# arnaucube/go-snark-study

Measured on AMD Instinct MI355X. Metric: Groth16 constraints/sec (prove) at 2^20 R1CS, higher is better.
Workload: dtype u32 (9x29-bit Montgomery limbs of the 254-bit BN128 fields)

## Files before the change

go-snark-study_amd/csrc/knobs.h:

```cpp
#pragma once
#include <cerrno>
#include <cstdlib>

namespace gs {

inline bool knob_parse(const char* name, long lo, long hi, long multiple_of, bool pow2, long& out) {
  const char* s = getenv(name);
  if (!s || !*s) return false;
  char* end = nullptr;
  errno = 0;
  const long v = strtol(s, &end, 10);
  if (errno != 0 || end == s || *end != '\0') return false;
  if (v < lo || v > hi) return false;
  if (multiple_of > 1 && v % multiple_of != 0) return false;
  if (pow2 && (v <= 0 || (v & (v - 1)) != 0)) return false;
  out = v;
  return true;
}

inline bool run_flag(const char* name) { return getenv(name) != nullptr; }
inline long run_knob(const char* name, long dflt, long lo, long hi) {
  long v = dflt;
  return knob_parse(name, lo, hi, 1, false, v) ? v : dflt;
}

#ifdef GS_DEV_KNOBS
inline bool dev_flag(const char* name) { return getenv(name) != nullptr; }
inline long dev_knob(const char* name, long dflt, long lo, long hi, long multiple_of = 1, bool pow2 = false) {
  long v = dflt;
  return knob_parse(name, lo, hi, multiple_of, pow2, v) ? v : dflt;
}
inline double dev_knob_f(const char* name, double dflt, double lo, double hi) {
  const char* s = getenv(name);
  if (!s || !*s) return dflt;
  char* end = nullptr;
  const double v = strtod(s, &end);
  return (end == s || *end != '\0' || !(v >= lo && v <= hi)) ? dflt : v;
}
#else
inline bool dev_flag(const char*) { return false; }
inline long dev_knob(const char*, long dflt, long, long, long = 1, bool = false) { return dflt; }
inline double dev_knob_f(const char*, double dflt, double, double) { return dflt; }
#endif

}
```

go-snark-study_amd/csrc/msm.hip:

```cpp
#include "msm.h"
#include "hostcopy.h"

#include <algorithm>
#include <cmath>
#include <cstdlib>
#include <future>
#include <type_traits>

#include "msm_kernels.h"

namespace gs {

static_assert(sizeof(G1Xyzz) == PointIO<FqTag>::kXyzzWords * 4, "G1 XYZZ must be raw limbs");
static_assert(sizeof(G2Xyzz) == PointIO<Fq2Tag>::kXyzzWords * 4, "G2 XYZZ must be raw limbs");

static inline dim3 grid1(size_t n, int block = 256) { return dim3((unsigned)((n + block - 1) / block)); }

int choose_window_bits(uint32_t n, int forced) {
  if (forced >= 8 && forced <= kMaxWindowBits) return forced;
  static const double per_bucket = dev_knob_f("GS_WINDOW_COST_BUCKET", 6.0, 0.0, 64.0);
  static const int auto_max = (int)dev_knob("GS_AUTO_MAX_C", 17, 8, kMaxWindowBits);
  int best = 8;
  double best_cost = 1e300;
  for (int c = 8; c <= std::min(kMaxWindowBits, std::max(8, auto_max)); ++c) {
    const int W = 254 / c + 1;
    const double cost = (double)n * W + per_bucket * (double)(1u << (c - 1));
    if (cost < best_cost) { best_cost = cost; best = c; }
  }
  return best;
}

int choose_window_bits_free(uint32_t n, int forced) {
  if (forced) return std::min(kMaxFreeWindowBits, std::max(kMinFreeWindowBits, forced));
  static const double per_bucket = dev_knob_f("GS_WINDOW_COST_BUCKET_FREE", 3.0, 0.0, 64.0);
  int best = kMinFreeWindowBits;
  double best_cost = 1e300;
  for (int c = kMinFreeWindowBits; c <= kMaxFreeWindowBits; ++c) {
    const int W = 254 / c + 1;
    const double cost = (double)W * ((double)n + per_bucket * (double)(1u << (c - 1)));
    if (cost < best_cost) { best_cost = cost; best = c; }
  }
  return best;
}

static void exclusive_scan(Ctx& c, PlanBuffers& pb, const uint32_t* in, uint32_t* out, uint32_t n) {
  const uint32_t ntiles = (n + kScanTile - 1) / kScanTile;
  pb.tiles.ensure((size_t)ntiles * 4);
  pb.total.ensure(4);
  hipLaunchKernelGGL(k_scan_tiles, dim3(ntiles), dim3(kScanBlock), 0, c.stream, in, out, pb.tiles.as<uint32_t>(), n);
  hipLaunchKernelGGL(k_scan_tile_sums, dim3(1), dim3(1024), 0, c.stream, pb.tiles.as<uint32_t>(), ntiles, pb.total.as<uint32_t>());
  hipLaunchKernelGGL(k_scan_add, dim3(ntiles), dim3(kScanBlock), 0, c.stream, out, pb.tiles.as<uint32_t>(), n);
}

struct MsmState {
  PlanBuffers plan_slots[3 * Ctx::kSlots];
  DevBuf table_scratch;
  DevBuf table_scratch_bg;
  DevBuf upload_scratch;
  DevBuf upload_flag;
  bool lds_attr_set = false;
};
static MsmState& msm_state(Ctx& c) { return c.state<MsmState>(c.msm_state); }

static uint32_t choose_chunk(uint64_t entries, uint32_t nbuckets, const std::vector<LaunchShape>& users) {
  static const int forced = (int)dev_knob("GS_CHUNK", 0, 4, 1024, 4);
  if (forced >= 4 && forced % 4 == 0) return (uint32_t)forced;
  static const int forced_h = (int)dev_knob("GS_CHUNK_H", 0, 4, 1024, 4);
  if (forced_h && users.size() == 1 && users[0].njobs == 1 && !users[0].g2) return (uint32_t)forced_h;
  uint32_t chunk = entries >= (1ull << 27) ? 64u : entries >= (1ull << 23) ? 32u : 16u;
  while (chunk < 1024u && entries / std::max<uint32_t>(nbuckets, 1u) > 32ull * chunk) chunk *= 2;
  return chunk;
}

static uint32_t part_min_ranges() {
  static const uint32_t v = (uint32_t)dev_knob("GS_PART_MIN_R", 4, 2, 64);
  return v;
}
bool plan_partitions_first(int cbits) {
// ... 28 lines not shown
  plan.B = 1u << (plan.c - 1);
  plan.nbuckets = table_free ? (uint32_t)plan.W * plan.B : plan.B;
  plan.chunk = choose_chunk((uint64_t)n * plan.W, plan.nbuckets, users);
  plan.maxchunks = (uint32_t)(((size_t)n * plan.W + plan.chunk - 1) / plan.chunk) + 1;
  const size_t ncount = (size_t)plan.nbuckets + 1;
  PlanParams pp{};
  pp.n = n; pp.c = plan.c; pp.W = plan.W; pp.B = plan.B;
  pp.R = std::max<uint32_t>(1u, plan.B >> kRangeLog);
  pp.tf = table_free ? 1u : 0u;
  {
    const uint32_t want = std::max<uint32_t>(1u, 256u / (plan.W * pp.R));
    const uint32_t by_size = std::max<uint32_t>(1u, (n + 16383u) / 16384u);
    const uint32_t by_mem = std::max<uint32_t>(1u, (uint32_t)((64ull << 20) / ((uint64_t)plan.B * plan.W * 4)));
    pp.S = std::max<uint32_t>(1u, std::min(std::min<uint32_t>(16u, std::max<uint32_t>(want, 1u)), std::min(by_size, by_mem)));
    if (pp.R == 1 && !table_free) pp.S = std::max<uint32_t>(1u, std::min<uint32_t>(16u, by_size));
  }
  pp.slice = (n + pp.S - 1) / pp.S;
  pp.stride = (n + 63u) & ~63u;
  const bool wide = plan_partitions_first(plan.c);
  if (wide && term_index) throw HipError{hipErrorInvalidValue, "plans over a term list cannot be sorted partition-first (plan_partitions_first)", __LINE__};
  const uint32_t nparts = (uint32_t)plan.W * pp.R;
  if (wide && nparts > kMaxParts) throw HipError{hipErrorInvalidValue, "too many (window, range) partitions", __LINE__};
  if (!wide) pb.digits.ensure((size_t)std::max<uint32_t>(pp.stride, 64u) * plan.W * sizeof(digit_t));
  else {
    pb.recs.ensure(std::max<size_t>((size_t)n * plan.W, 1) * 8);
    pb.parts.ensure((size_t)(3 * kMaxParts + 4) * 4);
  }
  pb.hist.ensure((size_t)plan.B * plan.W * pp.S * 4);
  pb.totals.ensure(ncount * 4);
  pb.offsets.ensure(ncount * 4);
  pb.entries.ensure(((size_t)plan.maxchunks + 1) * plan.chunk * 4);
  pb.chunk_bucket.ensure((size_t)plan.maxchunks * 4);
  pb.heavy_list.ensure((size_t)plan.nbuckets * 4);
  pb.counters.ensure(16);
  const size_t lds = (size_t)std::min<uint32_t>(plan.B, kRangeBuckets) * 4;
  static const int sort_block = (int)dev_knob("GS_SORT_BLOCK", kSortBlock, 64, kSortBlock, 64);
  if (!ms.lds_attr_set) {
    GS_HIP(hipFuncSetAttribute(reinterpret_cast<const void*>(k_hist), hipFuncAttributeMaxDynamicSharedMemorySize, 128 * 1024));
    GS_HIP(hipFuncSetAttribute(reinterpret_cast<const void*>(k_scatter), hipFuncAttributeMaxDynamicSharedMemorySize, 128 * 1024));
    GS_HIP(hipFuncSetAttribute(reinterpret_cast<const void*>(k_hist_part), hipFuncAttributeMaxDynamicSharedMemorySize, 128 * 1024));
    GS_HIP(hipFuncSetAttribute(reinterpret_cast<const void*>(k_scatter_part), hipFuncAttributeMaxDynamicSharedMemorySize, 128 * 1024));
    ms.lds_attr_set = true;
  }
  GS_HIP(hipMemsetAsync(pb.totals.as<uint32_t>() + plan.nbuckets, 0, 4, c.stream));
  GS_HIP(hipMemsetAsync(pb.counters.p, 0, 16, c.stream));
  uint32_t* part_count = pb.parts.as<uint32_t>();
  uint32_t* part_base = part_count ? part_count + kMaxParts : nullptr;
  uint32_t* part_cursor = part_count ? part_base + kMaxParts + 4 : nullptr;
  if (n > 0 && wide) {
    GS_HIP(hipMemsetAsync(part_count, 0, (size_t)nparts * 4, c.stream));
    hipLaunchKernelGGL(k_part_count, grid1(n, kPartBlock), dim3(kPartBlock), 0, c.stream, scalars_dev, pp, part_count);
    hipLaunchKernelGGL(k_part_scan, dim3(1), dim3(64), 0, c.stream, part_count, nparts, part_base, part_cursor);
    hipLaunchKernelGGL(k_part_scatter, grid1(n, kPartBlock * kPartPerThread), dim3(kPartBlock), 0, c.stream, scalars_dev, pp, part_base, part_cursor,
                       pb.recs.as<uint2>());
    hipLaunchKernelGGL(k_hist_part, dim3(8 * pp.S * ((nparts + 7) / 8)), dim3(sort_block), lds, c.stream, pb.recs.as<uint2>(), part_base, pp, pb.hist.as<uint32_t>());
    hipLaunchKernelGGL(k_colscan, grid1(plan.B), dim3(256), 0, c.stream, pb.hist.as<uint32_t>(), pp, pb.totals.as<uint32_t>());
  } else if (n > 0) {
    hipLaunchKernelGGL(k_digits, grid1(n), dim3(256), 0, c.stream, scalars_dev, pp, pb.digits.as<digit_t>(), term_index, index_bias);
    hipLaunchKernelGGL(k_hist, dim3(plan.W, pp.S, pp.R), dim3(sort_block), lds, c.stream, pb.digits.as<digit_t>(), pp, pb.hist.as<uint32_t>());
    if (table_free) hipLaunchKernelGGL(k_colscan_windows, grid1(plan.nbuckets), dim3(256), 0, c.stream, pb.hist.as<uint32_t>(), pp, pb.totals.as<uint32_t>());
    else hipLaunchKernelGGL(k_colscan, grid1(plan.B), dim3(256), 0, c.stream, pb.hist.as<uint32_t>(), pp, pb.totals.as<uint32_t>());
  } else {
    GS_HIP(hipMemsetAsync(pb.totals.p, 0, ncount * 4, c.stream));
  }
  exclusive_scan(c, pb, pb.totals.as<uint32_t>(), pb.offsets.as<uint32_t>(), (uint32_t)ncount);
  if (n > 0) {
    if (wide) hipLaunchKernelGGL(k_scatter_part, dim3(8 * pp.S * ((nparts + 7) / 8)), dim3(sort_block), lds, c.stream, pb.recs.as<uint2>(), part_base, pp,
                                 pb.hist.as<uint32_t>(), pb.offsets.as<uint32_t>(), pb.entries.as<uint32_t>());
    else hipLaunchKernelGGL(k_scatter, dim3(plan.W, pp.S, pp.R), dim3(sort_block), lds, c.stream, pb.digits.as<digit_t>(), pp, pb.hist.as<uint32_t>(),
                            pb.offsets.as<uint32_t>(), pb.entries.as<uint32_t>(), term_index, index_bias);
    hipLaunchKernelGGL(k_chunk_map, grid1(plan.nbuckets), dim3(256), 0, c.stream, pb.offsets.as<uint32_t>(), plan.nbuckets, plan.chunk,
                       pb.chunk_bucket.as<uint32_t>(), pb.heavy_list.as<uint32_t>(), pb.counters.as<uint32_t>());
  }
  GS_HIP(hipGetLastError());
  plan.offsets = pb.offsets.as<uint32_t>();
  plan.entries = pb.entries.as<uint32_t>();
  plan.chunk_bucket = pb.chunk_bucket.as<uint32_t>();
  plan.heavy_list = pb.heavy_list.as<uint32_t>();
  plan.heavy_count = pb.counters.as<uint32_t>();
}

template <class T>
static void enqueue_table_slabs(hipStream_t stream, DevBuf& scratch, const uint32_t* src, size_t n, int cbits, DevBuf& rows, size_t first, size_t last,
                                size_t slab) {
  const int W = 254 / cbits + 1;
  if (first >= last) return;
  static const bool per_row = dev_flag("GS_TABLE_PER_ROW");
  if (per_row || W <= 2) {
    if (first == 0) hipLaunchKernelGGL(k_build_table<T>, grid1(n), dim3(256), 0, stream, src, (uint32_t)n, cbits, W, rows.as<uint32_t>());
  } else {
    constexpr size_t sw = PointIO<T>::kXyzzWords + PointIO<T>::kXyzzWords / 4;
    slab = std::min<size_t>(std::max<size_t>(slab, 1), n);
    scratch.ensure(slab * (size_t)(W - 1) * sw * 4);
    for (size_t at = first; at < last; at += slab) {
// ... 205 lines not shown
  if (out_bytes > Ctx::kPinnedBytes) throw HipError{hipErrorInvalidValue, "MSM result staging too small", __LINE__};
  p.stats_off = out_bytes - stats_bytes;
  AccJobs jobs{};
  DevBuf& outb = c.ws_out[ws_base % Ctx::kWsSets];
  outb.ensure(pair_bytes + final_bytes + stats_bytes);
  uint32_t* finals = outb.as<uint32_t>() + pair_bytes / 4;
  uint32_t* stats = finals + final_bytes / 4;
  for (int j = 0; j < njobs; ++j) {
    const BaseTable* t = bases[j].table;
    const uint32_t* points = nullptr;
    uint32_t row_stride = 0;
    if (plan.table_free) {
      if (!bases[j].points || bases[j].off + plan.n > bases[j].npoints)
        throw HipError{hipErrorInvalidValue, "MSM base array does not cover the plan", __LINE__};
      points = bases[j].points + bases[j].off * aw;
    } else {
      if (!t || t->c != plan.c || !t->rows.p || bases[j].off + plan.n > t->n)
        throw HipError{hipErrorInvalidValue, "MSM base table does not match the plan", __LINE__};
      points = t->rows.as<uint32_t>() + bases[j].off * aw;
      row_stride = (uint32_t)t->n;
    }
    DevBuf& bk = c.ws_buckets[(ws_base + j) % Ctx::kWsSets];
    DevBuf& mg = c.ws_chunks[(ws_base + j) % Ctx::kWsSets];
    DevBuf& pt = c.ws_partials[(ws_base + j) % Ctx::kWsSets];
    bk.ensure((size_t)plan.nbuckets * pw * 4);
    mg.ensure((size_t)plan.nbuckets * pw * 4);
    pt.ensure((size_t)plan.maxchunks * 2 * pw * 4);
    jobs.j[j] = AccJob{points, row_stride, bk.as<uint32_t>(), pt.as<uint32_t>(),
                       pt.as<uint32_t>() + (size_t)plan.maxchunks * pw, mg.as<uint32_t>(),
                       outb.as<uint32_t>() + (size_t)j * nblk * 2 * pw, finals + (size_t)j * pw};
  }
  p.tacc = std::make_shared<PhaseTimer>(c.stream);
  p.tker = std::make_shared<PhaseTimer>(c.stream);
  hipLaunchKernelGGL(k_bucket_accumulate<T>, dim3((plan.maxchunks + kAccBlock - 1) / kAccBlock, njobs), dim3(kAccBlock), 0, c.stream,
                     jobs, plan.offsets, plan.entries, plan.chunk_bucket, plan.nbuckets, plan.chunk);
  p.tker->stop();
  p.tacc->stop();
  hipStream_t ts = tail_stream ? tail_stream : c.stream;
  if (ts != c.stream) {
    hipEvent_t ev;
    GS_HIP(hipEventCreateWithFlags(&ev, hipEventDisableTiming));
    GS_HIP(hipEventRecord(ev, c.stream));
    GS_HIP(hipStreamWaitEvent(ts, ev, 0));
    GS_HIP(hipEventDestroy(ev));
  }
  p.tred = std::make_shared<PhaseTimer>(ts);
  static const long alone_below_log2 = dev_knob("GS_TAIL_ALONE_LOG2", 19, 0, 32);
  const bool alone = plan.n < (1ull << alone_below_log2);
  auto launch_tails = [&](auto alone_tag) {
    constexpr bool kAlone = decltype(alone_tag)::value;
    hipLaunchKernelGGL((k_heavy_combine<T, kAlone>), dim3(64, njobs), dim3(kHeavyBlock), 0, ts,
                       jobs, plan.offsets, plan.heavy_list, plan.heavy_count, plan.chunk);
    hipLaunchKernelGGL((k_heavy_finish<T, kAlone>), dim3(16, njobs), dim3(kHeavyBlock), 0, ts,
                       jobs, plan.offsets, plan.heavy_list, plan.heavy_count, plan.chunk);
    hipLaunchKernelGGL((k_bucket_combine<T, kAlone>), dim3((plan.nbuckets + 255) / 256, njobs), dim3(256), 0, ts, jobs, plan.offsets, plan.nbuckets,
                       plan.chunk, plan.heavy_count, stats);
    hipLaunchKernelGGL((k_block_reduce<T, kAlone>), dim3(nblk, njobs), dim3(kReduceBlock), 0, ts, jobs, plan.nbuckets, L);
    if (p.folded) {
      int log2_span = 0;
      while ((1u << log2_span) < (uint32_t)kReduceBlock * (uint32_t)L) ++log2_span;
      hipLaunchKernelGGL((k_pair_reduce<T, kAlone>), dim3(1, njobs), dim3(kReduceBlock), 0, ts, jobs, nblk, log2_span);
    }
  };
  if (alone) launch_tails(std::true_type{}); else launch_tails(std::false_type{});
  GS_HIP(hipGetLastError());
  GS_HIP(hipMemcpyAsync(c.pinned[slot], p.folded ? (const void*)finals : outb.p, out_bytes, hipMemcpyDeviceToHost, ts));
  p.pinned_slot = c.pinned[slot];
// ... 213 lines not shown
```

go-snark-study_amd/csrc/msm_kernels.h:

```cpp
#pragma once
#include <hip/hip_runtime.h>
#include <stdint.h>

#include "ec.h"
#include "point_io.h"

namespace gs {

struct PlanParams {
  uint32_t n;
  int c;
  int W;
  uint32_t B;
  uint32_t S;
  uint32_t slice;
  uint32_t stride;
  uint32_t R;
  uint32_t tf;
};
constexpr uint32_t kRangeLog = 15;
constexpr uint32_t kRangeBuckets = 1u << kRangeLog;

GS_HD int32_t next_digit(const uint32_t (&k)[8], const PlanParams& pp, int w, uint32_t& carry) {
  uint32_t raw = scalar_bits(k, w * pp.c, pp.c) + carry;
// ... 28 lines not shown
  if (i < n) {
    uint32_t acc = 0;
    if (a) for (uint32_t k = 0; k < wa; ++k) acc |= a[(size_t)i * wa + k];
    if (b) for (uint32_t k = 0; k < wb; ++k) acc |= b[(size_t)i * wb + k];
    finite = acc != 0;
  }
  if (finite) { atomicOr(&mask[i >> 5], 1u << (i & 31u)); atomicAdd(count, 1u); }
}

constexpr int kSortBlock = 1024;

__global__ void __launch_bounds__(kSortBlock) k_hist(const digit_t* __restrict__ digits, PlanParams pp, uint32_t* __restrict__ hist) {
  wave_priority<GS_PRIO_PLAN>();
  extern __shared__ uint32_t sh[];
  const uint32_t w = blockIdx.x, s = blockIdx.y, r = blockIdx.z;
  const uint32_t nb = min(pp.B, kRangeBuckets), base = r << kRangeLog;
  for (uint32_t b = threadIdx.x; b < nb; b += blockDim.x) sh[b] = 0;
  __syncthreads();
  const uint32_t lo = s * pp.slice, hi = min(pp.n, lo + pp.slice);
  const digit_t* row = digits + (size_t)w * pp.stride;
  const int32_t zero = (int32_t)pp.B - 1;
  for (uint32_t i = lo + threadIdx.x; i < hi; i += blockDim.x) {
    const int32_t d = (int32_t)row[i] - zero;
    if (d != 0) {
      const uint32_t b = (uint32_t)(d < 0 ? -d : d) - 1u;
      if ((b >> kRangeLog) == r) atomicAdd(&sh[b - base], 1u);
    }
  }
  __syncthreads();
  uint32_t* out = hist + ((size_t)w * pp.S + s) * pp.B + base;
  for (uint32_t b = threadIdx.x; b < nb; b += blockDim.x) out[b] = sh[b];
}

__global__ void __launch_bounds__(256) k_colscan(uint32_t* __restrict__ hist, PlanParams pp, uint32_t* __restrict__ totals) {
  wave_priority<GS_PRIO_PLAN>();
  const uint32_t b = blockIdx.x * blockDim.x + threadIdx.x;
  if (b >= pp.B) return;
  uint32_t* col = hist + b;
  const uint32_t nq = (uint32_t)pp.W * pp.S;
  uint32_t run = 0;
  for (uint32_t q = 0; q < nq; ++q) { const uint32_t t = col[(size_t)q * pp.B]; col[(size_t)q * pp.B] = run; run += t; }
  totals[b] = run;
}

__global__ void __launch_bounds__(256) k_colscan_windows(uint32_t* __restrict__ hist, PlanParams pp, uint32_t* __restrict__ totals) {
  wave_priority<GS_PRIO_PLAN>();
  const uint32_t i = blockIdx.x * blockDim.x + threadIdx.x;
  if (i >= (uint32_t)pp.W * pp.B) return;
  const uint32_t w = i / pp.B, b = i % pp.B;
  uint32_t* col = hist + (size_t)w * pp.S * pp.B + b;
  uint32_t run = 0;
  for (uint32_t q = 0; q < pp.S; ++q) { const uint32_t t = col[(size_t)q * pp.B]; col[(size_t)q * pp.B] = run; run += t; }
  totals[i] = run;
}

__global__ void __launch_bounds__(kSortBlock) k_scatter(const digit_t* __restrict__ digits, PlanParams pp, const uint32_t* __restrict__ hist,
                                                         const uint32_t* __restrict__ offsets, uint32_t* __restrict__ entries,
                                                         const uint32_t* __restrict__ term_index, uint32_t index_bias) {
  wave_priority<GS_PRIO_PLAN>();
  extern __shared__ uint32_t sh[];
  const uint32_t w = blockIdx.x, s = blockIdx.y, r = blockIdx.z;
  const uint32_t nb = min(pp.B, kRangeBuckets), base = r << kRangeLog;
  const uint32_t* pre = hist + ((size_t)w * pp.S + s) * pp.B + base;
  const uint32_t* off = offsets + (pp.tf ? (size_t)w * pp.B : (size_t)0);
  for (uint32_t b = threadIdx.x; b < nb; b += blockDim.x) sh[b] = off[base + b] + pre[b];
  __syncthreads();
  const uint32_t lo = s * pp.slice, hi = min(pp.n, lo + pp.slice);
  const digit_t* row = digits + (size_t)w * pp.stride;
  const int32_t zero = (int32_t)pp.B - 1;
  for (uint32_t i = lo + threadIdx.x; i < hi; i += blockDim.x) {
    const int32_t d = (int32_t)row[i] - zero;
    if (d != 0) {
      const uint32_t b = (uint32_t)(d < 0 ? -d : d) - 1u;
      if ((b >> kRangeLog) == r) {
        const uint32_t pos = atomicAdd(&sh[b - base], 1u);
        const uint32_t id = term_index ? term_index[i] - index_bias : i;
        entries[pos] = id | (w << kWindowShift) | (d < 0 ? kSignBit : 0u);
      }
    }
  }
// ... 156 lines not shown
#pragma unroll
  for (int j = 0; j < kScanPerThread; ++j) { if (base + j < n) out[base + j] = run; run += v[j]; }
  if (threadIdx.x == kScanBlock - 1) tile_sums[blockIdx.x] = sh[threadIdx.x];
}

__global__ void __launch_bounds__(1024) k_scan_tile_sums(uint32_t* __restrict__ tile_sums, uint32_t ntiles, uint32_t* __restrict__ total) {
  wave_priority<GS_PRIO_PLAN>();
  __shared__ uint32_t sh[1024];
  const uint32_t per = (ntiles + 1023u) / 1024u;
  const uint32_t b0 = threadIdx.x * per;
  uint32_t sum = 0;
  for (uint32_t j = 0; j < per; ++j) if (b0 + j < ntiles) sum += tile_sums[b0 + j];
  sh[threadIdx.x] = sum;
  __syncthreads();
  for (int off = 1; off < 1024; off <<= 1) {
    uint32_t t = (threadIdx.x >= (uint32_t)off) ? sh[threadIdx.x - off] : 0u;
    __syncthreads();
    sh[threadIdx.x] += t;
    __syncthreads();
  }
  uint32_t run = sh[threadIdx.x] - sum;
  for (uint32_t j = 0; j < per; ++j) if (b0 + j < ntiles) { uint32_t t = tile_sums[b0 + j]; tile_sums[b0 + j] = run; run += t; }
  if (threadIdx.x == 1023) *total = sh[1023];
}

__global__ void __launch_bounds__(kScanBlock) k_scan_add(uint32_t* __restrict__ out, const uint32_t* __restrict__ tile_sums, uint32_t n) {
  wave_priority<GS_PRIO_PLAN>();
  const uint32_t base = blockIdx.x * kScanTile + threadIdx.x * kScanPerThread;
  const uint32_t add = tile_sums[blockIdx.x];
#pragma unroll
  for (int j = 0; j < kScanPerThread; ++j) if (base + j < n) out[base + j] += add;
}

constexpr uint32_t kHeavySpan = 64;

__global__ void __launch_bounds__(256) k_chunk_map(const uint32_t* __restrict__ offsets, uint32_t nbuckets, uint32_t chunk,
                                                    uint32_t* __restrict__ chunk_bucket, uint32_t* __restrict__ heavy_list,
                                                    uint32_t* __restrict__ heavy_count) {
  wave_priority<GS_PRIO_PLAN>();
  const uint32_t b = blockIdx.x * blockDim.x + threadIdx.x;
  if (b >= nbuckets) return;
  const uint32_t o0 = offsets[b], o1 = offsets[b + 1];
  if (o1 == o0) return;
  const uint32_t t0 = (o0 + chunk - 1) / chunk, t1 = (o1 + chunk - 1) / chunk;
  for (uint32_t t = t0; t < t1; ++t) chunk_bucket[t] = b;
  if ((o1 - 1) / chunk - o0 / chunk > kHeavySpan) {
    heavy_list[atomicAdd(heavy_count, 1u)] = b;
  }
}

struct AccJob {
  const uint32_t* table;
  uint32_t row_stride;
  uint32_t* buckets;
  uint32_t* heads;
  uint32_t* tails;
  uint32_t* merged;
  uint32_t* out;
  uint32_t* final_out;
};
constexpr int kMaxJobs = 8;
struct AccJobs { AccJob j[kMaxJobs]; };

template <class T> struct AccTuning;
#ifndef GS_G1_WAVES
#define GS_G1_WAVES 3
#endif
#ifndef GS_G1_PREFETCH
#define GS_G1_PREFETCH 1
#endif
#ifndef GS_G2_TOUCH
#define GS_G2_TOUCH 0
#endif
template <> struct AccTuning<FqTag> { static constexpr int kMinWaves = GS_G1_WAVES; static constexpr bool kRegisterPrefetch = GS_G1_PREFETCH != 0; static constexpr bool kTouch = true; };
#ifndef GS_G2_WAVES
#define GS_G2_WAVES 2
#endif
#ifndef GS_G2_PREFETCH
#define GS_G2_PREFETCH 0
#endif
template <> struct AccTuning<Fq2Tag> { static constexpr int kMinWaves = GS_G2_WAVES; static constexpr bool kRegisterPrefetch = GS_G2_PREFETCH != 0; static constexpr bool kTouch = GS_G2_TOUCH != 0; };

#ifndef GS_ACC_BLOCK
#define GS_ACC_BLOCK 256
#endif
constexpr int kAccBlock = GS_ACC_BLOCK;
template <class T>
__global__ void __launch_bounds__(kAccBlock, AccTuning<T>::kMinWaves) k_bucket_accumulate(AccJobs jobs, const uint32_t* __restrict__ offsets,
                                                            const uint32_t* __restrict__ entries,
                                                            const uint32_t* __restrict__ chunk_bucket, uint32_t nbuckets, uint32_t chunk) {
  constexpr int pw = PointIO<T>::kXyzzWords;
  constexpr int aw = PointIO<T>::kAffineWords;
  const uint32_t t = blockIdx.x * blockDim.x + threadIdx.x;
  const uint32_t total = offsets[nbuckets];
  const uint32_t beg = t * chunk;
  if (beg >= total) return;
  const uint32_t end = min(beg + chunk, total);
  const AccJob job = jobs.j[blockIdx.y];
  uint32_t b = chunk_bucket[t];
  uint32_t bend = offsets[b + 1];
  bool started_before = offsets[b] < beg;
  constexpr bool kTight = GS_PAIR != 0 && T::kWords != 8;
  using Acc = std::conditional_t<kTight, XyzzAcc<T>, Xyzz<T>>;
  auto acc_inf = [] { if constexpr (kTight) return xyzz_acc_inf<T>(); else return xyzz_inf<T>(); };
  auto acc_store = [](uint32_t* p, const Acc& a) { if constexpr (kTight) store_xyzz<T>(p, to_xyzz(a)); else store_xyzz<T>(p, a); };
  Acc acc = acc_inf();
  const uint4* e4 = reinterpret_cast<const uint4*>(entries + beg);
  constexpr bool kPre = AccTuning<T>::kRegisterPrefetch;
  uint4 q = e4[0];
  uint32_t v = q.x;
  uint32_t nb = b;
  const uint32_t* np = job.table + ((size_t)((v >> kWindowShift) & 31u) * job.row_stride + (v & kIndexMask)) * aw;
  RawAffine<T> nextp;
  uint32_t touch = 0;
  if constexpr (kPre) nextp = load_raw_affine<T>(np);
  for (uint32_t e = beg; e < end; ++e) {
    const uint32_t cur = v;
    const uint32_t* cp = np;
    RawAffine<T> curp;
    if constexpr (kPre) curp = nextp;
    if (e >= bend) {
// ... 399 lines not shown
```

go-snark-study_amd/csrc/poly.hip:

```cpp
#include "poly.h"

#include <algorithm>
#include <vector>

#include "poly_kernels.h"

namespace gs {

static inline dim3 grid1(size_t n, int block = 256) { return dim3((unsigned)((n + block - 1) / block)); }

int ceil_log2(size_t n) {
  int l = 0;
  while (((size_t)1 << l) < n) ++l;
  return l;
}

static FrConst to_const(const Fe<ModR, 2>& a) {
  FrConst c;
  for (int i = 0; i < NL; ++i) c.l[i] = a.l[i];
  return c;
}
Fe<ModR, 2> fr_from_words_mont(const uint64_t w[4]) {
  uint32_t u[8];
  for (int i = 0; i < 4; ++i) { u[2 * i] = (uint32_t)w[i]; u[2 * i + 1] = (uint32_t)(w[i] >> 32); }
// ... 197 lines not shown
  }
  GS_HIP(hipGetLastError());
}

void divisor_init(Ctx& c, Divisor& d, const uint32_t* b_std_dev, size_t nb) {
  d.nb = nb;
  d.b_std.alloc(nb * 32);
  GS_HIP(hipMemcpyAsync(d.b_std.p, b_std_dev, nb * 32, hipMemcpyDeviceToDevice, c.stream));
  d.k = 0;
  d.logn_spec = 0;
  d.k_spec = 0;
}

static void divisor_ensure(Ctx& c, Divisor& d, size_t k) {
  if (k <= d.k) return;
  const size_t fl = std::min(d.nb, k);
  DevBuf f(fl * 32);
  hipLaunchKernelGGL(k_copy_reversed, grid1(fl), dim3(256), 0, c.stream, d.b_std.as<uint32_t>(), (uint32_t)(d.nb - fl), (uint32_t)fl,
                     f.as<uint32_t>(), (uint32_t)fl);
  poly_canon_dev(c, f.as<uint32_t>(), fl, 1);
  d.inv_rev_mont.alloc(k * 32);
  poly_inv_series_dev(c, f.as<uint32_t>(), fl, k, d.inv_rev_mont.as<uint32_t>());
  GS_HIP(hipStreamSynchronize(c.stream));
  d.k = k;
  d.logn_spec = 0;
}

void poly_quotient_dev(Ctx& c, Divisor& d, const uint32_t* a, size_t na, uint32_t* quo) {
  if (na < d.nb) return;
  const size_t k = na - d.nb + 1;
  divisor_ensure(c, d, k);
  const int logn = ceil_log2(2 * k - 1);
  const size_t N = (size_t)1 << logn;
  if (d.logn_spec != logn || d.k_spec != k) {
    d.inv_spec.alloc(N * 32);
    copy_padded(c, d.inv_rev_mont.as<uint32_t>(), k, d.inv_spec.as<uint32_t>(), N);
    ntt_forward(c, d.inv_spec.as<uint32_t>(), logn, logn);
    d.logn_spec = logn;
    d.k_spec = k;
  }
  poly_state(c).ws_a.ensure(N * 32);
  uint32_t* A = poly_state(c).ws_a.as<uint32_t>();
  hipLaunchKernelGGL(k_copy_reversed, grid1(N), dim3(256), 0, c.stream, a, (uint32_t)(na - k), (uint32_t)k, A, (uint32_t)N);
  ntt_forward(c, A, logn, logn);
  if (logn >= 1) ntt_inverse_unscaled_of_product_n(c, A, N, logn, d.inv_spec.as<uint32_t>());
  else hipLaunchKernelGGL(k_pw_mul, grid1(N), dim3(256), 0, c.stream, A, d.inv_spec.as<uint32_t>(), A, (uint32_t)N);
  poly_state(c).ws_b.ensure(k * 32);
  hipLaunchKernelGGL(k_copy_reversed, grid1(k), dim3(256), 0, c.stream, A, 0u, (uint32_t)k, poly_state(c).ws_b.as<uint32_t>(), (uint32_t)k);
  hipLaunchKernelGGL(k_pw_mul_const, grid1(k), dim3(256), 0, c.stream, poly_state(c).ws_b.as<uint32_t>(), inv_n_const(logn, 0), quo, (uint32_t)k);
  GS_HIP(hipGetLastError());
}


static void prefix_products(Ctx& c, int mode, uint32_t top, uint32_t count, uint32_t* out, Fe<ModR, 2>* last_host) {
  const uint32_t ntiles = (count + kPpTile - 1) / kPpTile;
  DevBuf tiles((size_t)ntiles * 32);
  hipLaunchKernelGGL(k_pp_tiles, dim3(ntiles), dim3(kPpBlock), 0, c.stream, mode, top, count, out, tiles.as<uint32_t>());
  if (ntiles > 1) {
    hipLaunchKernelGGL(k_pp_tile_scan, dim3(1), dim3(1024), 0, c.stream, tiles.as<uint32_t>(), ntiles);
    hipLaunchKernelGGL(k_pp_apply, grid1(count), dim3(256), 0, c.stream, out, tiles.as<uint32_t>(), count);
  }
  GS_HIP(hipGetLastError());
  if (last_host) {
    uint32_t w[8];
    GS_HIP(hipMemcpyAsync(w, out + (size_t)(count - 1) * 8, 32, hipMemcpyDeviceToHost, c.stream));
    GS_HIP(hipStreamSynchronize(c.stream));
    *last_host = reduce2(unpack32<ModR>(w));
  }
  GS_HIP(hipStreamSynchronize(c.stream));
}
static void ensure_factorials(Ctx& c, size_t top) {
  PolyState& ps = poly_state(c);
  if (top <= ps.fact_top) return;
  top = std::max<size_t>(top, 2 * ps.fact_top);
  if (top >= (1ull << 31)) throw HipError{hipErrorInvalidValue, "factorial table too large", __LINE__};
  DevBuf fwd(top * 32), rev(top * 32);
  Fe<ModR, 2> top_fact;
  prefix_products(c, 0, (uint32_t)top, (uint32_t)top, fwd.as<uint32_t>(), &top_fact);
  prefix_products(c, 1, (uint32_t)top, (uint32_t)top, rev.as<uint32_t>(), nullptr);
  ps.fact.alloc((top + 1) * 32);
  ps.invfact.alloc((top + 1) * 32);
  hipLaunchKernelGGL(k_fact_tables, grid1(top + 1), dim3(256), 0, c.stream, fwd.as<uint32_t>(), rev.as<uint32_t>(), to_const(inv(top_fact)), (uint32_t)top,
// ... 302 lines not shown
```

go-snark-study_amd/csrc/poly_kernels.h:

```cpp
#pragma once
#include <hip/hip_runtime.h>
#include <stdint.h>

#include "fp29.h"

namespace gs {

using Fr6 = Fe<ModR, 6>;
using Fr2 = Fe<ModR, 2>;

GS_HD Fr6 load_fr(const uint32_t* p) {
  const uint4* q = reinterpret_cast<const uint4*>(p);
  const uint4 lo = q[0], hi = q[1];
  uint32_t w[8] = {lo.x, lo.y, lo.z, lo.w, hi.x, hi.y, hi.z, hi.w};
  return unpack32<ModR>(w);
}
GS_HD void store_fr(uint32_t* p, const Fr2& a) {
  Fr2 x = a;
  carry_full(x);
  Fe<ModR, 1> y;
#pragma unroll
  for (int i = 0; i < NL; ++i) y.l[i] = x.l[i];
  uint32_t w[8];
  pack32<ModR>(y, w);
// ... 108 lines not shown
  } else {
    Fe<ModR, B> b[N];
#pragma unroll
    for (int k = 0; k < N; ++k)
#pragma unroll
      for (int l = 0; l < NL; ++l) b[k].l[l] = x[k].b[l];
    if constexpr (N == 2) dots2<ModR>(dot_of(b[0], w[0]), dot_of(b[1], w[1]), t[0], t[1]);
    else t[0] = mul_lazy(b[0], w[0]);
  }
#pragma unroll
  for (int k = 0; k < N; ++k) {
    uint32_t p[NL], m[NL];
#pragma unroll
    for (int l = 0; l < NL; ++l) { p[l] = x[k].a[l] + t[k].l[l]; m[l] = x[k].a[l] + (ModR::tbias(3, l) - t[k].l[l]); }
    static_assert(ModR::tbias_k(3) == 3, "the DIT bound table (B + 2, B + 3) assumes the 3r bias");
    if (!lazy_out) {
      Fe<ModR, B + 3> pp, mm;
#pragma unroll
      for (int l = 0; l < NL; ++l) { pp.l[l] = p[l]; mm.l[l] = m[l]; }
      carry_save(pp); carry_save(mm);
#pragma unroll
      for (int l = 0; l < NL; ++l) { p[l] = pp.l[l]; m[l] = mm.l[l]; }
    }
#pragma unroll
    for (int l = 0; l < NL; ++l) { x[k].a[l] = p[l]; x[k].b[l] = m[l]; }
  }
}
template <int N>
GS_HD void ntt_dit_butterfly(int step, int nsteps, Bfly (&x)[N], const Fe<ModR, 1> (&w)[N], bool trivial) {
  const bool lazy_out = (step & 1) == 0 && step + 1 < nsteps;
  ntt_dit_step<20, N>(x, w, true, lazy_out, trivial);
}

constexpr int kNttLoadPlain = 0, kNttLoadScaled = 1, kNttLoadWeighed = 2;
struct NttLoadAux {
  const uint32_t* aux0;
  const uint32_t* aux1;
  uint32_t n;
  uint32_t logN;
};

template <bool kInverse, int kLoad = kNttLoadPlain>
__global__ void __launch_bounds__(256) k_ntt_pass(uint32_t* __restrict__ x, const uint32_t* __restrict__ tw, int tw_logn, int s_lo, int k, int clog, NttLoadAux aux) {
  wave_priority<GS_PRIO_POLY>();
  __shared__ uint32_t sh[NL * kNttTile];
  const uint32_t R = 1u << k, C = 1u << clog, E = R << clog;
  const uint32_t tile = blockIdx.x;
  size_t base;
  uint32_t qstride, cstride;
  if (s_lo == 0) { base = (size_t)tile * E; qstride = 1; cstride = R; }
  else {
    const uint32_t chunks = (1u << s_lo) >> clog;
    const uint32_t hi = tile / chunks, lc = tile - hi * chunks;
    base = ((size_t)hi << (s_lo + k)) + ((size_t)lc << clog); qstride = 1u << s_lo; cstride = 1;
  }
  for (uint32_t e = threadIdx.x; e < E; e += 256) {
    uint32_t q, cc;
    if (s_lo == 0) { q = e & (R - 1); cc = e >> k; } else { cc = e & (C - 1); q = e >> clog; }
    const size_t gi = base + (size_t)q * qstride + (size_t)cc * cstride;
    Fr2 v;
    if constexpr (kLoad == kNttLoadWeighed) {
      const size_t vec = gi >> aux.logN;
      const uint32_t j = (uint32_t)(gi & (((size_t)1 << aux.logN) - 1));
      if (j < aux.n) v = mul(load_fr(aux.aux0 + (vec * aux.n + j) * 8), load_fr(aux.aux1 + (size_t)j * 8));
      else v = fe_zero<ModR, 2>();
    } else if constexpr (kLoad == kNttLoadScaled) {
      v = mul(reduce2(load_fr(x + gi * 8)), load_fr(aux.aux0 + (gi & (((size_t)1 << aux.logN) - 1)) * 8));
    } else {
      v = reduce2(load_fr(x + gi * 8));
    }
    const uint32_t le = (q << clog) + cc;
#pragma unroll
    for (int l = 0; l < NL; ++l) sh[l * kNttTile + le] = v.l[l];
  }
  __syncthreads();
  auto twiddle_at = [&](uint32_t q0, uint32_t cc, int b) {
    const size_t gi = base + (size_t)q0 * qstride + (size_t)cc * cstride;
    const int s = s_lo + b;
    const uint32_t j = (uint32_t)gi & ((1u << s) - 1u);
    return load_twiddle(tw + ((size_t)j << (tw_logn - 1 - s)) * kTwWords);
  };
  int step = 0;
  for (; step < k; ++step) {
    const int b = kInverse ? step : k - 1 - step;
    const bool trivial = (s_lo + b) == 0;
    auto slots = [&](uint32_t u, uint32_t& e0, uint32_t& e1, uint32_t& q0, uint32_t& cc) {
      cc = u & (C - 1);
      const uint32_t qq = u >> clog;
      q0 = ((qq >> b) << (b + 1)) | (qq & ((1u << b) - 1u));
      e0 = (q0 << clog) + cc; e1 = e0 + ((1u << b) << clog);
    };
    uint32_t u = threadIdx.x;
    for (; u + 256 < E / 2; u += 512) {
      uint32_t e0[2], e1[2], q0[2], cc[2];
      slots(u, e0[0], e1[0], q0[0], cc[0]);
      slots(u + 256, e0[1], e1[1], q0[1], cc[1]);
      Fe<ModR, 1> w[2];
      if (!trivial) { w[0] = twiddle_at(q0[0], cc[0], b); w[1] = twiddle_at(q0[1], cc[1], b); }
      Bfly x[2];
#pragma unroll
      for (int t = 0; t < 2; ++t)
#pragma unroll
        for (int l = 0; l < NL; ++l) { x[t].a[l] = sh[l * kNttTile + e0[t]]; x[t].b[l] = sh[l * kNttTile + e1[t]]; }
      if constexpr (kInverse) ntt_dit_butterfly<2>(step, k, x, w, trivial);
      else ntt_dif_butterfly<2>(step, x, w, trivial);
#pragma unroll
      for (int t = 0; t < 2; ++t)
#pragma unroll
        for (int l = 0; l < NL; ++l) { sh[l * kNttTile + e0[t]] = x[t].a[l]; sh[l * kNttTile + e1[t]] = x[t].b[l]; }
    }
    for (; u < E / 2; u += 256) {
      uint32_t e0, e1, q0, cc;
      slots(u, e0, e1, q0, cc);
      Fe<ModR, 1> w[1];
      if (!trivial) w[0] = twiddle_at(q0, cc, b);
      Bfly x[1];
#pragma unroll
      for (int l = 0; l < NL; ++l) { x[0].a[l] = sh[l * kNttTile + e0]; x[0].b[l] = sh[l * kNttTile + e1]; }
      if constexpr (kInverse) ntt_dit_butterfly<1>(step, k, x, w, trivial);
      else ntt_dif_butterfly<1>(step, x, w, trivial);
#pragma unroll
      for (int l = 0; l < NL; ++l) { sh[l * kNttTile + e0] = x[0].a[l]; sh[l * kNttTile + e1] = x[0].b[l]; }
    }
    __syncthreads();
  }
  for (uint32_t e = threadIdx.x; e < E; e += 256) {
    uint32_t q, cc;
    if (s_lo == 0) { q = e & (R - 1); cc = e >> k; } else { cc = e & (C - 1); q = e >> clog; }
    const uint32_t le = (q << clog) + cc;
    Fe<ModR, kNttEndBound> v;
#pragma unroll
    for (int l = 0; l < NL; ++l) v.l[l] = sh[l * kNttTile + le];
    store_fr(x + (base + (size_t)q * qstride + (size_t)cc * cstride) * 8, reduce2(v));
  }
}

__global__ void __launch_bounds__(256) k_pw_mul(const uint32_t* __restrict__ a, const uint32_t* __restrict__ b,
                                                 uint32_t* __restrict__ out, uint32_t n) {
  wave_priority<GS_PRIO_POLY>();
  const uint32_t i = blockIdx.x * blockDim.x + threadIdx.x;
  if (i >= n) return;
  store_fr(out + (size_t)i * 8, mul(load_fr(a + (size_t)i * 8), load_fr(b + (size_t)i * 8)));
}
__global__ void __launch_bounds__(256) k_pw_mul_const(const uint32_t* __restrict__ a, FrConst k, uint32_t* __restrict__ out, uint32_t n) {
  wave_priority<GS_PRIO_POLY>();
  const uint32_t i = blockIdx.x * blockDim.x + threadIdx.x;
  if (i >= n) return;
  store_fr(out + (size_t)i * 8, mul(load_fr(a + (size_t)i * 8), from_const(k)));
}
__global__ void __launch_bounds__(256) k_addsub(const uint32_t* __restrict__ a, uint32_t na, const uint32_t* __restrict__ b, uint32_t nb,
                                                 int subtract, uint32_t* __restrict__ out, uint32_t n) {
  const uint32_t i = blockIdx.x * blockDim.x + threadIdx.x;
  if (i >= n) return;
  const Fr6 x = (i < na) ? load_fr(a + (size_t)i * 8) : fe_zero<ModR, 6>();
  const Fr6 y = (i < nb) ? load_fr(b + (size_t)i * 8) : fe_zero<ModR, 6>();
  if (subtract) store_fr(out + (size_t)i * 8, reduce2(sub(x, y)));
  else store_fr(out + (size_t)i * 8, reduce2(add(x, y)));
}
__global__ void __launch_bounds__(256) k_copy_reversed(const uint32_t* __restrict__ src, uint32_t first, uint32_t count,
                                                        uint32_t* __restrict__ dst, uint32_t total) {
  wave_priority<GS_PRIO_POLY>();
  const uint32_t i = blockIdx.x * blockDim.x + threadIdx.x;
  if (i >= total) return;
  uint4* d = reinterpret_cast<uint4*>(dst + (size_t)i * 8);
  if (i < count) {
    const uint4* s = reinterpret_cast<const uint4*>(src + (size_t)(first + count - 1 - i) * 8);
// ... 398 lines not shown
```

Before: 120.4 million.

## Fuse side-chain kernels: single-block scan, colscan clears, reversed NTT load/store

Adds a default-on side-chain mode with several independent changes. Small exclusive scans run as one single-block kernel instead of three launches, and the plan counter clears are folded into the colscan kernel instead of separate memsets. Polynomial division folds the reversed copies and the 1/N scaling into the NTT passes via new reversed load and store modes, with the scale folded into the cached inverse spectrum. The accumulate block size is also split per curve group. These cut launches and extra memory passes on small side stages, at the risk of subtle index or correctness issues in the fused NTT path.

```diff
diff --git a/go-snark-study_amd/csrc/knobs.h b/go-snark-study_amd/csrc/knobs.h
--- a/go-snark-study_amd/csrc/knobs.h
+++ b/go-snark-study_amd/csrc/knobs.h
@@ -24,6 +24,11 @@
   return knob_parse(name, lo, hi, 1, false, v) ? v : dflt;
 }
 
+inline bool side_chain_fused() {
+  static const bool on = run_knob("GS_SIDE_CHAIN", 1, 0, 1) == 1;
+  return on;
+}
+
 #ifdef GS_DEV_KNOBS
 inline bool dev_flag(const char* name) { return getenv(name) != nullptr; }
 inline long dev_knob(const char* name, long dflt, long lo, long hi, long multiple_of = 1, bool pow2 = false) {
diff --git a/go-snark-study_amd/csrc/msm.hip b/go-snark-study_amd/csrc/msm.hip
--- a/go-snark-study_amd/csrc/msm.hip
+++ b/go-snark-study_amd/csrc/msm.hip
@@ -43,7 +43,13 @@
   return best;
 }
 
+constexpr uint32_t kScanOneMax = 1u << 17;
 static void exclusive_scan(Ctx& c, PlanBuffers& pb, const uint32_t* in, uint32_t* out, uint32_t n) {
+  static const uint32_t one_max = (uint32_t)dev_knob("GS_SCAN_ONE_MAX", kScanOneMax, 0, 1 << 24);
+  if (side_chain_fused() && n <= one_max) {
+    hipLaunchKernelGGL(k_scan_one, dim3(1), dim3(kScanOneBlock), 0, c.stream, in, out, n);
+    return;
+  }
   const uint32_t ntiles = (n + kScanTile - 1) / kScanTile;
   pb.tiles.ensure((size_t)ntiles * 4);
   pb.total.ensure(4);
@@ -138,7 +144,7 @@
   pb.entries.ensure(((size_t)plan.maxchunks + 1) * plan.chunk * 4);
   pb.chunk_bucket.ensure((size_t)plan.maxchunks * 4);
   pb.heavy_list.ensure((size_t)plan.nbuckets * 4);
-  pb.counters.ensure(16);
+  pb.counters.ensure(kPlanCounterWords * 4);
   const size_t lds = (size_t)std::min<uint32_t>(plan.B, kRangeBuckets) * 4;
   static const int sort_block = (int)dev_knob("GS_SORT_BLOCK", kSortBlock, 64, kSortBlock, 64);
   if (!ms.lds_attr_set) {
@@ -148,8 +154,12 @@
     GS_HIP(hipFuncSetAttribute(reinterpret_cast<const void*>(k_scatter_part), hipFuncAttributeMaxDynamicSharedMemorySize, 128 * 1024));
     ms.lds_attr_set = true;
   }
-  GS_HIP(hipMemsetAsync(pb.totals.as<uint32_t>() + plan.nbuckets, 0, 4, c.stream));
-  GS_HIP(hipMemsetAsync(pb.counters.p, 0, 16, c.stream));
+  const bool clear_in_colscan = side_chain_fused() && n > 0 && !wide;
+  uint32_t* clear = clear_in_colscan ? pb.counters.as<uint32_t>() : nullptr;
+  if (!clear_in_colscan) {
+    GS_HIP(hipMemsetAsync(pb.totals.as<uint32_t>() + plan.nbuckets, 0, 4, c.stream));
+    GS_HIP(hipMemsetAsync(pb.counters.p, 0, 16, c.stream));
+  }
   uint32_t* part_count = pb.parts.as<uint32_t>();
   uint32_t* part_base = part_count ? part_count + kMaxParts : nullptr;
   uint32_t* part_cursor = part_count ? part_base + kMaxParts + 4 : nullptr;
@@ -160,12 +170,12 @@
     hipLaunchKernelGGL(k_part_scatter, grid1(n, kPartBlock * kPartPerThread), dim3(kPartBlock), 0, c.stream, scalars_dev, pp, part_base, part_cursor,
                        pb.recs.as<uint2>());
     hipLaunchKernelGGL(k_hist_part, dim3(8 * pp.S * ((nparts + 7) / 8)), dim3(sort_block), lds, c.stream, pb.recs.as<uint2>(), part_base, pp, pb.hist.as<uint32_t>());
-    hipLaunchKernelGGL(k_colscan, grid1(plan.B), dim3(256), 0, c.stream, pb.hist.as<uint32_t>(), pp, pb.totals.as<uint32_t>());
+    hipLaunchKernelGGL(k_colscan, grid1(plan.B), dim3(256), 0, c.stream, pb.hist.as<uint32_t>(), pp, pb.totals.as<uint32_t>(), nullptr);
   } else if (n > 0) {
     hipLaunchKernelGGL(k_digits, grid1(n), dim3(256), 0, c.stream, scalars_dev, pp, pb.digits.as<digit_t>(), term_index, index_bias);
     hipLaunchKernelGGL(k_hist, dim3(plan.W, pp.S, pp.R), dim3(sort_block), lds, c.stream, pb.digits.as<digit_t>(), pp, pb.hist.as<uint32_t>());
-    if (table_free) hipLaunchKernelGGL(k_colscan_windows, grid1(plan.nbuckets), dim3(256), 0, c.stream, pb.hist.as<uint32_t>(), pp, pb.totals.as<uint32_t>());
-    else hipLaunchKernelGGL(k_colscan, grid1(plan.B), dim3(256), 0, c.stream, pb.hist.as<uint32_t>(), pp, pb.totals.as<uint32_t>());
+    if (table_free) hipLaunchKernelGGL(k_colscan_windows, grid1(plan.nbuckets), dim3(256), 0, c.stream, pb.hist.as<uint32_t>(), pp, pb.totals.as<uint32_t>(), clear);
+    else hipLaunchKernelGGL(k_colscan, grid1(plan.B), dim3(256), 0, c.stream, pb.hist.as<uint32_t>(), pp, pb.totals.as<uint32_t>(), clear);
   } else {
     GS_HIP(hipMemsetAsync(pb.totals.p, 0, ncount * 4, c.stream));
   }
@@ -437,7 +447,8 @@
   }
   p.tacc = std::make_shared<PhaseTimer>(c.stream);
   p.tker = std::make_shared<PhaseTimer>(c.stream);
-  hipLaunchKernelGGL(k_bucket_accumulate<T>, dim3((plan.maxchunks + kAccBlock - 1) / kAccBlock, njobs), dim3(kAccBlock), 0, c.stream,
+  constexpr uint32_t acc_block = AccTuning<T>::kBlock;
+  hipLaunchKernelGGL(k_bucket_accumulate<T>, dim3((plan.maxchunks + acc_block - 1) / acc_block, njobs), dim3(acc_block), 0, c.stream,
                      jobs, plan.offsets, plan.entries, plan.chunk_bucket, plan.nbuckets, plan.chunk);
   p.tker->stop();
   p.tacc->stop();
diff --git a/go-snark-study_amd/csrc/msm_kernels.h b/go-snark-study_amd/csrc/msm_kernels.h
--- a/go-snark-study_amd/csrc/msm_kernels.h
+++ b/go-snark-study_amd/csrc/msm_kernels.h
@@ -84,9 +84,15 @@
   for (uint32_t b = threadIdx.x; b < nb; b += blockDim.x) out[b] = sh[b];
 }
 
-__global__ void __launch_bounds__(256) k_colscan(uint32_t* __restrict__ hist, PlanParams pp, uint32_t* __restrict__ totals) {
+constexpr int kPlanCounterWords = 4;
+GS_HD void plan_clear(uint32_t* __restrict__ totals, uint32_t nbuckets, uint32_t* __restrict__ clear) {
+  totals[nbuckets] = 0;
+  for (int i = 0; i < kPlanCounterWords; ++i) clear[i] = 0;
+}
+__global__ void __launch_bounds__(256) k_colscan(uint32_t* __restrict__ hist, PlanParams pp, uint32_t* __restrict__ totals, uint32_t* __restrict__ clear) {
   wave_priority<GS_PRIO_PLAN>();
   const uint32_t b = blockIdx.x * blockDim.x + threadIdx.x;
+  if (b == 0 && clear) plan_clear(totals, pp.B, clear);
   if (b >= pp.B) return;
   uint32_t* col = hist + b;
   const uint32_t nq = (uint32_t)pp.W * pp.S;
@@ -95,9 +101,10 @@
   totals[b] = run;
 }
 
-__global__ void __launch_bounds__(256) k_colscan_windows(uint32_t* __restrict__ hist, PlanParams pp, uint32_t* __restrict__ totals) {
+__global__ void __launch_bounds__(256) k_colscan_windows(uint32_t* __restrict__ hist, PlanParams pp, uint32_t* __restrict__ totals, uint32_t* __restrict__ clear) {
   wave_priority<GS_PRIO_PLAN>();
   const uint32_t i = blockIdx.x * blockDim.x + threadIdx.x;
+  if (i == 0 && clear) plan_clear(totals, (uint32_t)pp.W * pp.B, clear);
   if (i >= (uint32_t)pp.W * pp.B) return;
   const uint32_t w = i / pp.B, b = i % pp.B;
   uint32_t* col = hist + (size_t)w * pp.S * pp.B + b;
@@ -320,6 +327,49 @@
   for (int j = 0; j < kScanPerThread; ++j) if (base + j < n) out[base + j] += add;
 }
 
+constexpr int kScanOneBlock = 1024;
+constexpr uint32_t kScanOneTile = kScanOneBlock * 4;
+__global__ void __launch_bounds__(kScanOneBlock) k_scan_one(const uint32_t* __restrict__ in, uint32_t* __restrict__ out, uint32_t n) {
+  wave_priority<GS_PRIO_PLAN>();
+  __shared__ uint32_t wsum[kScanOneBlock / 64];
+  const uint32_t lane = threadIdx.x & 63u, wave = threadIdx.x >> 6;
+  uint32_t carry = 0;
+  for (uint32_t base = 0; base < n; base += kScanOneTile) {
+    const uint32_t i = base + threadIdx.x * 4u;
+    uint32_t v[4] = {0u, 0u, 0u, 0u};
+    const bool full = i < n && n - i >= 4u;
+    if (full) {
+      const uint4 q = *reinterpret_cast<const uint4*>(in + i);
+      v[0] = q.x; v[1] = q.y; v[2] = q.z; v[3] = q.w;
+    } else {
+#pragma unroll
+      for (int j = 0; j < 4; ++j) if (i + j < n) v[j] = in[i + j];
+    }
+    const uint32_t sum = v[0] + v[1] + v[2] + v[3];
+    uint32_t incl = sum;
+#pragma unroll
+    for (int off = 1; off < 64; off <<= 1) {
+      const uint32_t t = __shfl_up(incl, off, 64);
+      if (lane >= (uint32_t)off) incl += t;
+    }
+    if (lane == 63u) wsum[wave] = incl;
+    __syncthreads();
+    uint32_t before = 0, tile_total = 0;
+#pragma unroll
+    for (uint32_t w = 0; w < kScanOneBlock / 64; ++w) { const uint32_t t = wsum[w]; if (w < wave) before += t; tile_total += t; }
+    const uint32_t run = carry + before + incl - sum;
+    if (full) {
+      *reinterpret_cast<uint4*>(out + i) = make_uint4(run, run + v[0], run + v[0] + v[1], run + v[0] + v[1] + v[2]);
+    } else {
+      uint32_t r = run;
+#pragma unroll
+      for (int j = 0; j < 4; ++j) { if (i + j < n) out[i + j] = r; r += v[j]; }
+    }
+    carry += tile_total;
+    __syncthreads();
+  }
+}
+
 constexpr uint32_t kHeavySpan = 64;
 
 __global__ void __launch_bounds__(256) k_chunk_map(const uint32_t* __restrict__ offsets, uint32_t nbuckets, uint32_t chunk,
@@ -351,6 +401,15 @@
 struct AccJobs { AccJob j[kMaxJobs]; };
 
 template <class T> struct AccTuning;
+#ifndef GS_ACC_BLOCK
+#define GS_ACC_BLOCK 256
+#endif
+#ifndef GS_G1_ACC_BLOCK
+#define GS_G1_ACC_BLOCK GS_ACC_BLOCK
+#endif
+#ifndef GS_G2_ACC_BLOCK
+#define GS_G2_ACC_BLOCK GS_ACC_BLOCK
+#endif
 #ifndef GS_G1_WAVES
 #define GS_G1_WAVES 3
 #endif
@@ -360,21 +419,25 @@
 #ifndef GS_G2_TOUCH
 #define GS_G2_TOUCH 0
 #endif
-template <> struct AccTuning<FqTag> { static constexpr int kMinWaves = GS_G1_WAVES; static constexpr bool kRegisterPrefetch = GS_G1_PREFETCH != 0; static constexpr bool kTouch = true; };
+template <> struct AccTuning<FqTag> {
+  static constexpr int kMinWaves = GS_G1_WAVES, kBlock = GS_G1_ACC_BLOCK;
+  static constexpr bool kRegisterPrefetch = GS_G1_PREFETCH != 0; static constexpr bool kTouch = true;
+};
 #ifndef GS_G2_WAVES
 #define GS_G2_WAVES 2
 #endif
 #ifndef GS_G2_PREFETCH
 #define GS_G2_PREFETCH 0
 #endif
-template <> struct AccTuning<Fq2Tag> { static constexpr int kMinWaves = GS_G2_WAVES; static constexpr bool kRegisterPrefetch = GS_G2_PREFETCH != 0; static constexpr bool kTouch = GS_G2_TOUCH != 0; };
-
-#ifndef GS_ACC_BLOCK
-#define GS_ACC_BLOCK 256
-#endif
-constexpr int kAccBlock = GS_ACC_BLOCK;
+template <> struct AccTuning<Fq2Tag> {
+  static constexpr int kMinWaves = GS_G2_WAVES, kBlock = GS_G2_ACC_BLOCK;
+  static constexpr bool kRegisterPrefetch = GS_G2_PREFETCH != 0; static constexpr bool kTouch = GS_G2_TOUCH != 0;
+};
+static_assert(AccTuning<FqTag>::kBlock % 64 == 0 && AccTuning<FqTag>::kBlock >= 64 && AccTuning<FqTag>::kBlock <= 1024, "GS_G1_ACC_BLOCK: whole waves, <= 1024 threads");
+static_assert(AccTuning<Fq2Tag>::kBlock % 64 == 0 && AccTuning<Fq2Tag>::kBlock >= 64 && AccTuning<Fq2Tag>::kBlock <= 1024, "GS_G2_ACC_BLOCK: whole waves, <= 1024 threads");
+
 template <class T>
-__global__ void __launch_bounds__(kAccBlock, AccTuning<T>::kMinWaves) k_bucket_accumulate(AccJobs jobs, const uint32_t* __restrict__ offsets,
+__global__ void __launch_bounds__(AccTuning<T>::kBlock, AccTuning<T>::kMinWaves) k_bucket_accumulate(AccJobs jobs, const uint32_t* __restrict__ offsets,
                                                             const uint32_t* __restrict__ entries,
                                                             const uint32_t* __restrict__ chunk_bucket, uint32_t nbuckets, uint32_t chunk) {
   constexpr int pw = PointIO<T>::kXyzzWords;
diff --git a/go-snark-study_amd/csrc/poly.hip b/go-snark-study_amd/csrc/poly.hip
--- a/go-snark-study_amd/csrc/poly.hip
+++ b/go-snark-study_amd/csrc/poly.hip
@@ -253,22 +253,51 @@
   divisor_ensure(c, d, k);
   const int logn = ceil_log2(2 * k - 1);
   const size_t N = (size_t)1 << logn;
+  const bool fused = side_chain_fused();
   if (d.logn_spec != logn || d.k_spec != k) {
     d.inv_spec.alloc(N * 32);
     copy_padded(c, d.inv_rev_mont.as<uint32_t>(), k, d.inv_spec.as<uint32_t>(), N);
     ntt_forward(c, d.inv_spec.as<uint32_t>(), logn, logn);
+    if (fused) hipLaunchKernelGGL(k_pw_mul_const, grid1(N), dim3(256), 0, c.stream, d.inv_spec.as<uint32_t>(), inv_n_const(logn, 0), d.inv_spec.as<uint32_t>(), (uint32_t)N);
     d.logn_spec = logn;
     d.k_spec = k;
   }
   poly_state(c).ws_a.ensure(N * 32);
   uint32_t* A = poly_state(c).ws_a.as<uint32_t>();
-  hipLaunchKernelGGL(k_copy_reversed, grid1(N), dim3(256), 0, c.stream, a, (uint32_t)(na - k), (uint32_t)k, A, (uint32_t)N);
-  ntt_forward(c, A, logn, logn);
-  if (logn >= 1) ntt_inverse_unscaled_of_product_n(c, A, N, logn, d.inv_spec.as<uint32_t>());
-  else hipLaunchKernelGGL(k_pw_mul, grid1(N), dim3(256), 0, c.stream, A, d.inv_spec.as<uint32_t>(), A, (uint32_t)N);
-  poly_state(c).ws_b.ensure(k * 32);
-  hipLaunchKernelGGL(k_copy_reversed, grid1(k), dim3(256), 0, c.stream, A, 0u, (uint32_t)k, poly_state(c).ws_b.as<uint32_t>(), (uint32_t)k);
-  hipLaunchKernelGGL(k_pw_mul_const, grid1(k), dim3(256), 0, c.stream, poly_state(c).ws_b.as<uint32_t>(), inv_n_const(logn, 0), quo, (uint32_t)k);
+  if (!fused) {
+    hipLaunchKernelGGL(k_copy_reversed, grid1(N), dim3(256), 0, c.stream, a, (uint32_t)(na - k), (uint32_t)k, A, (uint32_t)N);
+    ntt_forward(c, A, logn, logn);
+    if (logn >= 1) ntt_inverse_unscaled_of_product_n(c, A, N, logn, d.inv_spec.as<uint32_t>());
+    else hipLaunchKernelGGL(k_pw_mul, grid1(N), dim3(256), 0, c.stream, A, d.inv_spec.as<uint32_t>(), A, (uint32_t)N);
+    poly_state(c).ws_b.ensure(k * 32);
+    hipLaunchKernelGGL(k_copy_reversed, grid1(k), dim3(256), 0, c.stream, A, 0u, (uint32_t)k, poly_state(c).ws_b.as<uint32_t>(), (uint32_t)k);
+    hipLaunchKernelGGL(k_pw_mul_const, grid1(k), dim3(256), 0, c.stream, poly_state(c).ws_b.as<uint32_t>(), inv_n_const(logn, 0), quo, (uint32_t)k);
+    GS_HIP(hipGetLastError());
+    return;
+  }
+  const uint32_t* top = a + (na - k) * 8;
+  if (logn == 0) {
+    hipLaunchKernelGGL(k_pw_mul, grid1(1), dim3(256), 0, c.stream, top, d.inv_spec.as<uint32_t>(), quo, 1u);
+    GS_HIP(hipGetLastError());
+    return;
+  }
+  Twiddles& tw = ensure_twiddles(c, logn);
+  const std::vector<NttPass> sched = ntt_schedule(N, logn);
+  const NttLoadAux in_aux{top, nullptr, (uint32_t)k, (uint32_t)logn, nullptr, 0u};
+  const NttLoadAux mid_aux{d.inv_spec.as<uint32_t>(), nullptr, 0u, (uint32_t)logn, quo, (uint32_t)k};
+  for (size_t i = 0; i < sched.size(); ++i) {
+    const NttPass& p = sched[i];
+    if (i == 0) hipLaunchKernelGGL((k_ntt_pass<false, kNttLoadReversed>), dim3(p.ntiles), dim3(256), 0, c.stream, A, tw.fwd.as<uint32_t>(), tw.logn, p.s_lo, p.k, p.clog, in_aux);
+    else hipLaunchKernelGGL((k_ntt_pass<false, kNttLoadPlain>), dim3(p.ntiles), dim3(256), 0, c.stream, A, tw.fwd.as<uint32_t>(), tw.logn, p.s_lo, p.k, p.clog, NttLoadAux{});
+  }
+  for (size_t i = sched.size(); i-- > 0;) {
+    const NttPass& p = sched[i];
+    const bool first = i + 1 == sched.size(), last = i == 0;
+    if (first && last) hipLaunchKernelGGL((k_ntt_pass<true, kNttLoadScaled, kNttStoreReversed>), dim3(p.ntiles), dim3(256), 0, c.stream, A, tw.inv.as<uint32_t>(), tw.logn, p.s_lo, p.k, p.clog, mid_aux);
+    else if (first) hipLaunchKernelGGL((k_ntt_pass<true, kNttLoadScaled>), dim3(p.ntiles), dim3(256), 0, c.stream, A, tw.inv.as<uint32_t>(), tw.logn, p.s_lo, p.k, p.clog, mid_aux);
+    else if (last) hipLaunchKernelGGL((k_ntt_pass<true, kNttLoadPlain, kNttStoreReversed>), dim3(p.ntiles), dim3(256), 0, c.stream, A, tw.inv.as<uint32_t>(), tw.logn, p.s_lo, p.k, p.clog, mid_aux);
+    else hipLaunchKernelGGL((k_ntt_pass<true, kNttLoadPlain>), dim3(p.ntiles), dim3(256), 0, c.stream, A, tw.inv.as<uint32_t>(), tw.logn, p.s_lo, p.k, p.clog, NttLoadAux{});
+  }
   GS_HIP(hipGetLastError());
 }
 
diff --git a/go-snark-study_amd/csrc/poly_kernels.h b/go-snark-study_amd/csrc/poly_kernels.h
--- a/go-snark-study_amd/csrc/poly_kernels.h
+++ b/go-snark-study_amd/csrc/poly_kernels.h
@@ -164,15 +164,18 @@
   ntt_dit_step<20, N>(x, w, true, lazy_out, trivial);
 }
 
-constexpr int kNttLoadPlain = 0, kNttLoadScaled = 1, kNttLoadWeighed = 2;
+constexpr int kNttLoadPlain = 0, kNttLoadScaled = 1, kNttLoadWeighed = 2, kNttLoadReversed = 3;
+constexpr int kNttStorePlain = 0, kNttStoreReversed = 1;
 struct NttLoadAux {
   const uint32_t* aux0;
   const uint32_t* aux1;
   uint32_t n;
   uint32_t logN;
+  uint32_t* out;
+  uint32_t nout;
 };
 
-template <bool kInverse, int kLoad = kNttLoadPlain>
+template <bool kInverse, int kLoad = kNttLoadPlain, int kStore = kNttStorePlain>
 __global__ void __launch_bounds__(256) k_ntt_pass(uint32_t* __restrict__ x, const uint32_t* __restrict__ tw, int tw_logn, int s_lo, int k, int clog, NttLoadAux aux) {
   wave_priority<GS_PRIO_POLY>();
   __shared__ uint32_t sh[NL * kNttTile];
@@ -198,6 +201,9 @@
       else v = fe_zero<ModR, 2>();
     } else if constexpr (kLoad == kNttLoadScaled) {
       v = mul(reduce2(load_fr(x + gi * 8)), load_fr(aux.aux0 + (gi & (((size_t)1 << aux.logN) - 1)) * 8));
+    } else if constexpr (kLoad == kNttLoadReversed) {
+      if (gi < aux.n) v = reduce2(load_fr(aux.aux0 + ((size_t)aux.n - 1 - gi) * 8));
+      else v = fe_zero<ModR, 2>();
     } else {
       v = reduce2(load_fr(x + gi * 8));
     }
@@ -263,7 +269,12 @@
     Fe<ModR, kNttEndBound> v;
 #pragma unroll
     for (int l = 0; l < NL; ++l) v.l[l] = sh[l * kNttTile + le];
-    store_fr(x + (base + (size_t)q * qstride + (size_t)cc * cstride) * 8, reduce2(v));
+    const size_t gi = base + (size_t)q * qstride + (size_t)cc * cstride;
+    if constexpr (kStore == kNttStoreReversed) {
+      if (gi < aux.nout) store_fr(aux.out + ((size_t)aux.nout - 1 - gi) * 8, reduce2(v));
+    } else {
+      store_fr(x + gi * 8, reduce2(v));
+    }
   }
 }
 
```

Measured after the change: 119.4 million, median of 2. About the same (-0.8%).
